# openpsi-project/ReaLHF

Measured on AMD Instinct MI355X. Metric: PPO samples/sec (whole node), 4xLLaMA-7B actor/critic/ref/RM, higher is better.
Workload: dtype bf16; 1 GPU; model=4xllama-7b, global_batch=16, seq_len=640, prompt_len=128, gen_len=512, parallelism=dp1, ppo_n_minibatches=4

## Files before the change

### realhf_amd/ops/csrc/elementwise.hip

```cpp
#include "common.h"

template <typename T, bool CONJ>
__global__ void rope_kernel(
    const T* __restrict__ x, T* __restrict__ out,
    const float* __restrict__ cosb, const float* __restrict__ sinb,
    const long* __restrict__ pos, int total, int nh, int hd) {
  int hd2 = hd / 2;
  long n_quads = (long)total * nh * (hd2 / 4);
  for (long i = (long)blockIdx.x * blockDim.x + threadIdx.x; i < n_quads;
       i += (long)gridDim.x * blockDim.x) {
    int q = i % (hd2 / 4);
    long th = i / (hd2 / 4);
    int h = th % nh;
    long t = th / nh;
    int d0 = q * 4;
    const T* base = x + (t * nh + h) * (long)hd;
    T* obase = out + (t * nh + h) * (long)hd;
    long p = pos[t];
    float4v c = *(const float4v*)(cosb + p * hd2 + d0);
    float4v s = *(const float4v*)(sinb + p * hd2 + d0);
    short4v x1 = *(const short4v*)((const short*)base + d0);
    short4v x2 = *(const short4v*)((const short*)base + hd2 + d0);
    short o1[4], o2[4];
    #pragma unroll
// ... 51 lines not shown
                                  long tokens, int I) {
  long n = tokens * (I / 8);
  for (long i = (long)blockIdx.x * blockDim.x + threadIdx.x; i < n;
       i += (long)gridDim.x * blockDim.x) {
    long t = i / (I / 8);
    int d0 = (int)(i % (I / 8)) * 8;
    const T* g = gu + t * (2L * I) + d0;
    const T* u = g + I;
    short8 gv = *(const short8*)g;
    short8 uv = *(const short8*)u;
    short o[8];
    #pragma unroll
    for (int j = 0; j < 8; j++) {
      float gf = to_f32<T>(((const T*)&gv)[j]);
      float uf = to_f32<T>(((const T*)&uv)[j]);
      float s = gf / (1.f + __expf(-glu_sig_arg<GELU>(gf)));
      ((T*)o)[j] = from_f32<T>(s * uf);
    }
    *(short8*)(out + t * (long)I + d0) = *(short8*)o;
  }
}

template <typename T, bool GELU = false>
__global__ void swiglu_slab_kernel(const float* __restrict__ parts, int nks,
                                   T* __restrict__ out, long tokens, int I) {
  const long sstride = tokens * (2L * I);
  long n = tokens * (I / 8);
  for (long i = (long)blockIdx.x * blockDim.x + threadIdx.x; i < n;
       i += (long)gridDim.x * blockDim.x) {
    long t = i / (I / 8);
    int d0 = (int)(i % (I / 8)) * 8;
    const float* g = parts + t * (2L * I) + d0;
    const float* u = g + I;
    float gf[8], uf[8];
    #pragma unroll
    for (int j = 0; j < 8; j += 4) {
      *(float4v*)(gf + j) = *(const float4v*)(g + j);
      *(float4v*)(uf + j) = *(const float4v*)(u + j);
    }
    for (int s = 1; s < nks; s++) {
      #pragma unroll
      for (int j = 0; j < 8; j += 4) {
        float4v pg = *(const float4v*)(g + (long)s * sstride + j);
        float4v pu = *(const float4v*)(u + (long)s * sstride + j);
        #pragma unroll
        for (int q = 0; q < 4; q++) { gf[j + q] += pg[q]; uf[j + q] += pu[q]; }
      }
    }
    short o[8];
    #pragma unroll
    for (int j = 0; j < 8; j++) {
      float sg = gf[j] / (1.f + __expf(-glu_sig_arg<GELU>(gf[j])));
      ((T*)o)[j] = from_f32<T>(sg * uf[j]);
    }
    *(short8*)(out + t * (long)I + d0) = *(short8*)o;
  }
}

template <typename T, bool GELU = false>
__global__ void swiglu_bwd_kernel(const T* __restrict__ dy, const T* __restrict__ gu,
                                  T* __restrict__ dgu, long tokens, int I) {
  long n = tokens * (I / 8);
  for (long i = (long)blockIdx.x * blockDim.x + threadIdx.x; i < n;
       i += (long)gridDim.x * blockDim.x) {
    long t = i / (I / 8);
    int d0 = (int)(i % (I / 8)) * 8;
    const T* g = gu + t * (2L * I) + d0;
    const T* u = g + I;
    short8 gv = *(const short8*)g;
    short8 uv = *(const short8*)u;
    short8 dv = *(const short8*)(dy + t * (long)I + d0);
    short dg[8], du[8];
    #pragma unroll
    for (int j = 0; j < 8; j++) {
      float gf = to_f32<T>(((const T*)&gv)[j]);
      float uf = to_f32<T>(((const T*)&uv)[j]);
// ... 166 lines not shown
```

### realhf_amd/ops/csrc/rmsnorm.hip

```cpp
#include "common.h"

template <typename T, bool GEMMA>
DEVINL float norm_weight(T w) {
  if constexpr (GEMMA) return 1.0f + to_f32<T>(w);
  else return to_f32<T>(w);
}

template <typename T, int VEC, bool RESID = false, bool GEMMA = false>
__global__ void rmsnorm_fwd_kernel(
    const T* __restrict__ x, const T* __restrict__ w, T* __restrict__ out,
    float* __restrict__ rstd, int rows, int H, float eps,
    const T* __restrict__ resid = nullptr, T* __restrict__ sum_out = nullptr) {
  __shared__ float red[8];
  for (int row = blockIdx.x; row < rows; row += gridDim.x) {
    const T* xr = x + (long)row * H;
    T* yr = out + (long)row * H;
    float ss = 0.f;
    for (int i = threadIdx.x * VEC; i < H; i += blockDim.x * VEC) {
      T v[VEC];
      *(float4v*)v = *(const float4v*)(xr + i);
      if constexpr (RESID) {
        T r[VEC];
        *(float4v*)r = *(const float4v*)(resid + (long)row * H + i);
        #pragma unroll
        for (int j = 0; j < VEC; j++)
          v[j] = from_f32<T>(to_f32<T>(v[j]) + to_f32<T>(r[j]));
        *(float4v*)(sum_out + (long)row * H + i) = *(float4v*)v;
      }
      #pragma unroll
      for (int j = 0; j < VEC; j++) { float f = to_f32<T>(v[j]); ss += f * f; }
    }
    ss = wave_sum(ss);
    int wid = threadIdx.x / WAVE;
    int nw = blockDim.x / WAVE;
    if ((threadIdx.x & (WAVE - 1)) == 0) red[wid] = ss;
    __syncthreads();
    if (threadIdx.x < 8) {
      float v2 = (threadIdx.x < nw) ? red[threadIdx.x] : 0.f;
      for (int off = 4; off > 0; off >>= 1) v2 += __shfl_down(v2, off, 64);
      if (threadIdx.x == 0) red[0] = v2;
    }
    __syncthreads();
    float rs = rsqrtf(red[0] / H + eps);
    if (threadIdx.x == 0 && rstd) rstd[row] = rs;
    const T* src2 = RESID ? (sum_out + (long)row * H) : xr;
    for (int i = threadIdx.x * VEC; i < H; i += blockDim.x * VEC) {
      T v[VEC], wv[VEC], o[VEC];
      *(float4v*)v = *(const float4v*)(src2 + i);
      *(float4v*)wv = *(const float4v*)(w + i);
      #pragma unroll
      for (int j = 0; j < VEC; j++)
        o[j] = from_f32<T>(to_f32<T>(v[j]) * rs * norm_weight<T, GEMMA>(wv[j]));
      *(float4v*)(yr + i) = *(float4v*)o;
    }
    __syncthreads();
  }
}

template <typename T, int VEC, bool GEMMA = false>
__global__ void add_rmsnorm_slab_kernel(
    const float* __restrict__ parts, int nks, const T* __restrict__ resid,
    const T* __restrict__ w, T* __restrict__ out, T* __restrict__ sum_out,
    int rows, int H, float eps) {
  __shared__ float red[8];
  const long sstride = (long)rows * H;
  for (int row = blockIdx.x; row < rows; row += gridDim.x) {
// ... 4 lines not shown
      const float* pr = parts + (long)row * H + i;
      #pragma unroll
      for (int j = 0; j < VEC; j += 4)
        *(float4v*)(f + j) = *(const float4v*)(pr + j);
      for (int s = 1; s < nks; s++) {
        #pragma unroll
        for (int j = 0; j < VEC; j += 4) {
          float4v p = *(const float4v*)(pr + (long)s * sstride + j);
          #pragma unroll
          for (int q = 0; q < 4; q++) f[j + q] += p[q];
        }
      }
      T r[VEC], v[VEC];
      *(float4v*)r = *(const float4v*)(resid + (long)row * H + i);
      #pragma unroll
      for (int j = 0; j < VEC; j++) {
        float fv = f[j] + to_f32<T>(r[j]);
        v[j] = from_f32<T>(fv);
        float fq = to_f32<T>(v[j]);
        ss += fq * fq;
      }
      *(float4v*)(sum_out + (long)row * H + i) = *(float4v*)v;
    }
    ss = wave_sum(ss);
    int wid = threadIdx.x / WAVE;
    int nw = blockDim.x / WAVE;
    if ((threadIdx.x & (WAVE - 1)) == 0) red[wid] = ss;
    __syncthreads();
    if (threadIdx.x < 8) {
      float v2 = (threadIdx.x < nw) ? red[threadIdx.x] : 0.f;
      for (int off = 4; off > 0; off >>= 1) v2 += __shfl_down(v2, off, 64);
      if (threadIdx.x == 0) red[0] = v2;
    }
    __syncthreads();
    float rs = rsqrtf(red[0] / H + eps);
    const T* src2 = sum_out + (long)row * H;
    for (int i = threadIdx.x * VEC; i < H; i += blockDim.x * VEC) {
      T v[VEC], wv[VEC], o[VEC];
      *(float4v*)v = *(const float4v*)(src2 + i);
      *(float4v*)wv = *(const float4v*)(w + i);
      #pragma unroll
      for (int j = 0; j < VEC; j++)
        o[j] = from_f32<T>(to_f32<T>(v[j]) * rs * norm_weight<T, GEMMA>(wv[j]));
      *(float4v*)(yr + i) = *(float4v*)o;
    }
    __syncthreads();
  }
}

#define RMS_MAX_COLS 64
#define RMS_THREADS 256

template <typename T, int VEC, bool GEMMA = false>
__global__ void __launch_bounds__(GEMMA ? RMS_THREADS : 1024) rmsnorm_bwd_kernel(
    const T* __restrict__ dy, const T* __restrict__ x, const T* __restrict__ w,
    const float* __restrict__ rstd, T* __restrict__ dx,
    float* __restrict__ dw, int rows, int H) {
  __shared__ float red[8];
  float dwacc[RMS_MAX_COLS];
  #pragma unroll
  for (int j = 0; j < RMS_MAX_COLS; j++) dwacc[j] = 0.f;
  for (int row = blockIdx.x; row < rows; row += gridDim.x) {
    const T* dyr = dy + (long)row * H;
    const T* xr = x + (long)row * H;
    T* dxr = dx + (long)row * H;
    float rs = rstd[row];
    float dot = 0.f;
    for (int i = threadIdx.x * VEC; i < H; i += blockDim.x * VEC) {
      T a[VEC], b[VEC], c[VEC];
      *(float4v*)a = *(const float4v*)(dyr + i);
      *(float4v*)b = *(const float4v*)(w + i);
      *(float4v*)c = *(const float4v*)(xr + i);
      #pragma unroll
      for (int j = 0; j < VEC; j++)
        dot += to_f32<T>(a[j]) * norm_weight<T, GEMMA>(b[j]) * to_f32<T>(c[j]);
    }
    dot = wave_sum(dot);
    int wid = threadIdx.x / WAVE, nw = blockDim.x / WAVE;
    if ((threadIdx.x & (WAVE - 1)) == 0) red[wid] = dot;
    __syncthreads();
    if (threadIdx.x < 8) {
      float v2 = (threadIdx.x < nw) ? red[threadIdx.x] : 0.f;
      for (int off = 4; off > 0; off >>= 1) v2 += __shfl_down(v2, off, 64);
      if (threadIdx.x == 0) red[0] = v2;
    }
    __syncthreads();
    float k = red[0] * rs * rs * rs / H;
    if constexpr (GEMMA) {
      #pragma unroll
      for (int c = 0; c < RMS_MAX_COLS / VEC; c++) {
        int i = (c * RMS_THREADS + (int)threadIdx.x) * VEC;
        if (i >= H) continue;
        T a[VEC], b[VEC], cx[VEC], o[VEC];
        *(float4v*)a = *(const float4v*)(dyr + i);
        *(float4v*)b = *(const float4v*)(w + i);
        *(float4v*)cx = *(const float4v*)(xr + i);
        #pragma unroll
        for (int j = 0; j < VEC; j++) {
          float g = to_f32<T>(a[j]);
          float xv = to_f32<T>(cx[j]);
          o[j] = from_f32<T>(rs * norm_weight<T, true>(b[j]) * g - k * xv);
          dwacc[c * VEC + j] += g * xv * rs;
        }
        *(float4v*)(dxr + i) = *(float4v*)o;
      }
    } else {
      int slot = 0;
      for (int i = threadIdx.x * VEC; i < H; i += blockDim.x * VEC, slot += VEC) {
        T a[VEC], b[VEC], c[VEC], o[VEC];
        *(float4v*)a = *(const float4v*)(dyr + i);
// ... 21 lines not shown
      for (int j = 0; j < VEC; j++) dwrow[i + j] = dwacc[c * VEC + j];
    }
  } else {
    int slot = 0;
    for (int i = threadIdx.x * VEC; i < H; i += blockDim.x * VEC, slot += VEC) {
      #pragma unroll
      for (int j = 0; j < VEC; j++)
        if (slot + j < RMS_MAX_COLS) dwrow[i + j] = dwacc[slot + j];
    }
  }
}

template <bool GEMMA>
static std::vector<torch::Tensor> rmsnorm_fwd_impl(torch::Tensor x, torch::Tensor w,
                                                   double eps) {
  TORCH_CHECK(x.is_cuda() && x.is_contiguous());
  int H = x.size(-1);
  long rows = x.numel() / H;
  auto out = torch::empty_like(x);
  auto rstd = torch::empty({rows}, x.options().dtype(torch::kFloat));
  int vec = 16 / x.element_size();
  TORCH_CHECK(H % vec == 0, "hidden dim must be divisible by ", vec);
  int grid = (int)std::min<long>(rows, 2048);
  DISPATCH_BF16_FP16_FP32(x.scalar_type(), "rmsnorm_fwd", [&] {
    if (x.element_size() == 2) {
      hipLaunchKernelGGL((rmsnorm_fwd_kernel<scalar_t, 8, false, GEMMA>), dim3(grid), dim3(256), 0,
        cur_stream(), (const scalar_t*)x.data_ptr(), (const scalar_t*)w.data_ptr(),
        (scalar_t*)out.data_ptr(), rstd.data_ptr<float>(), (int)rows, H, (float)eps);
    } else {
      hipLaunchKernelGGL((rmsnorm_fwd_kernel<scalar_t, 4, false, GEMMA>), dim3(grid), dim3(256), 0,
        cur_stream(), (const scalar_t*)x.data_ptr(), (const scalar_t*)w.data_ptr(),
        (scalar_t*)out.data_ptr(), rstd.data_ptr<float>(), (int)rows, H, (float)eps);
    }
  });
  CHECK_CUDA_OK();
  return {out, rstd};
}

template <bool GEMMA>
static std::vector<torch::Tensor> add_rmsnorm_fwd_impl(torch::Tensor x,
                                                       torch::Tensor resid,
                                                       torch::Tensor w, double eps) {
  TORCH_CHECK(x.is_cuda() && x.is_contiguous() && resid.is_contiguous());
  int H = x.size(-1);
  long rows = resid.numel() / H;
  TORCH_CHECK(H % 8 == 0);
  auto out = torch::empty_like(resid);
  auto sum_out = torch::empty_like(resid);
  int grid = (int)std::min<long>(rows, 2048);
  if (x.dim() == 3 && x.scalar_type() == torch::kFloat) {
    TORCH_CHECK(resid.scalar_type() == torch::kBFloat16);
    TORCH_CHECK(x.size(1) * x.size(2) == rows * H);
    hipLaunchKernelGGL((add_rmsnorm_slab_kernel<bf16, 8, GEMMA>), dim3(grid),
      dim3(256), 0, cur_stream(), x.data_ptr<float>(), (int)x.size(0),
      (const bf16*)resid.data_ptr(), (const bf16*)w.data_ptr(),
      (bf16*)out.data_ptr(), (bf16*)sum_out.data_ptr(), (int)rows, H,
      (float)eps);
    CHECK_CUDA_OK();
    return {out, sum_out};
  }
  TORCH_CHECK(x.element_size() == 2);
  DISPATCH_BF16_FP16_FP32(x.scalar_type(), "add_rmsnorm", [&] {
    if constexpr (sizeof(scalar_t) == 2) {
      hipLaunchKernelGGL((rmsnorm_fwd_kernel<scalar_t, 8, true, GEMMA>), dim3(grid),
        dim3(256), 0, cur_stream(), (const scalar_t*)x.data_ptr(),
        (const scalar_t*)w.data_ptr(), (scalar_t*)out.data_ptr(),
        nullptr, (int)rows, H, (float)eps,
        (const scalar_t*)resid.data_ptr(), (scalar_t*)sum_out.data_ptr());
    }
  });
  CHECK_CUDA_OK();
  return {out, sum_out};
}

template <bool GEMMA>
static std::vector<torch::Tensor> rmsnorm_bwd_impl(torch::Tensor dy, torch::Tensor x,
                                                   torch::Tensor w,
                                                   torch::Tensor rstd) {
  int H = x.size(-1);
  TORCH_CHECK(H <= 256 * RMS_MAX_COLS, "rmsnorm_bwd supports hidden <= 16384");
  long rows = x.numel() / H;
  auto dx = torch::empty_like(x);
  int grid = (int)std::min<long>(rows, 512);
  auto dw32 = torch::zeros({grid, H}, x.options().dtype(torch::kFloat));
  DISPATCH_BF16_FP16_FP32(x.scalar_type(), "rmsnorm_bwd", [&] {
    if (x.element_size() == 2) {
      hipLaunchKernelGGL((rmsnorm_bwd_kernel<scalar_t, 8, GEMMA>), dim3(grid), dim3(RMS_THREADS), 0,
        cur_stream(), (const scalar_t*)dy.data_ptr(), (const scalar_t*)x.data_ptr(),
        (const scalar_t*)w.data_ptr(), rstd.data_ptr<float>(),
        (scalar_t*)dx.data_ptr(), dw32.data_ptr<float>(), (int)rows, H);
    } else {
// ... 34 lines not shown
```

### realhf_amd/ops/csrc/rope_decode.hip

```cpp
#include "common.h"
#include "fp8_e4m3.h"

template <bool SLAB, int FP8_HD = 0>
__global__ void rope_qkv_decode_kernel(
    const void* __restrict__ qkv_in,
    const bf16* __restrict__ bias,
    bf16* __restrict__ q_out,
    void* __restrict__ kcache,
    void* __restrict__ vcache,
    float* __restrict__ kscale,
    float* __restrict__ vscale,
    const int* __restrict__ cache_seqlens,
    const float* __restrict__ cosb, const float* __restrict__ sinb,
    int bs, int nq, int nkv, int hd, long maxlen, long qkv_stride,
    bool apply_rope, int nks) {
  const int nh = nq + 2 * nkv;
  const int hd2 = hd / 2;
  const long nwork = (long)bs * nh * (hd2 / 4);
  for (long i = (long)blockIdx.x * blockDim.x + threadIdx.x; i < nwork;
       i += (long)gridDim.x * blockDim.x) {
    const int quad = i % (hd2 / 4);
    const int h = (i / (hd2 / 4)) % nh;
    const int b = i / ((long)nh * (hd2 / 4));
    const int d0 = quad * 4;
    const int pos = max(cache_seqlens[b] - 1, 0);

    float4v f1, f2;
    if constexpr (SLAB) {
      const float* src =
          (const float*)qkv_in + (long)b * qkv_stride + (long)h * hd;
      const long sstride = (long)bs * qkv_stride;
      f1 = *(const float4v*)(src + d0);
      f2 = *(const float4v*)(src + hd2 + d0);
      for (int s = 1; s < nks; s++) {
        float4v p1 = *(const float4v*)(src + (long)s * sstride + d0);
        float4v p2 = *(const float4v*)(src + (long)s * sstride + hd2 + d0);
        #pragma unroll
        for (int j = 0; j < 4; j++) { f1[j] += p1[j]; f2[j] += p2[j]; }
      }
    } else {
      const bf16* src =
          (const bf16*)qkv_in + (long)b * qkv_stride + (long)h * hd;
      short4v x1 = *(const short4v*)((const short*)src + d0);
      short4v x2 = *(const short4v*)((const short*)src + hd2 + d0);
      #pragma unroll
      for (int j = 0; j < 4; j++) {
        f1[j] = __bfloat162float(((const bf16*)&x1)[j]);
        f2[j] = __bfloat162float(((const bf16*)&x2)[j]);
      }
    }
    if (bias) {
      short4v b1 = *(const short4v*)((const short*)bias + (long)h * hd + d0);
      short4v b2 = *(const short4v*)((const short*)bias + (long)h * hd + hd2 + d0);
      #pragma unroll
      for (int j = 0; j < 4; j++) {
        f1[j] += __bfloat162float(((const bf16*)&b1)[j]);
        f2[j] += __bfloat162float(((const bf16*)&b2)[j]);
      }
    }
    bf16* dst;
    bool rope = apply_rope;
    if (h < nq) {
      dst = q_out + ((long)b * nq + h) * hd;
    } else if (h < nq + nkv) {
      dst = (bf16*)kcache + (((long)b * maxlen + pos) * nkv + (h - nq)) * hd;
    } else {
      dst = (bf16*)vcache +
            (((long)b * maxlen + pos) * nkv + (h - nq - nkv)) * hd;
      rope = false;
    }
    short o1[4], o2[4];
    if (rope) {
      float4v c = *(const float4v*)(cosb + (long)pos * hd2 + d0);
      float4v s = *(const float4v*)(sinb + (long)pos * hd2 + d0);
      #pragma unroll
      for (int j = 0; j < 4; j++) {
        ((bf16*)o1)[j] = __float2bfloat16(f1[j] * c[j] - f2[j] * s[j]);
        ((bf16*)o2)[j] = __float2bfloat16(f2[j] * c[j] + f1[j] * s[j]);
      }
    } else {
      #pragma unroll
      for (int j = 0; j < 4; j++) {
        ((bf16*)o1)[j] = __float2bfloat16(f1[j]);
        ((bf16*)o2)[j] = __float2bfloat16(f2[j]);
      }
    }
    if constexpr (FP8_HD != 0) {
      if (h >= nq) {
        float amax = 0.f;
        #pragma unroll
        for (int j = 0; j < 4; j++)
          amax = fmaxf(amax, fmaxf(fabsf(bf2f(o1[j])), fabsf(bf2f(o2[j]))));
        amax = group_max<FP8_HD / 8>(amax);
        const float sc = e4m3_row_scale(amax);
        const bool is_k = h < nq + nkv;
        const int kvh = is_k ? h - nq : h - nq - nkv;
        unsigned char* cdst =
// ... 111 lines not shown
```

### realhf_amd/ops/csrc/skinny_gemm.hip

```cpp
#include "mfma.h"

#define SG_TN 64

template <int NT>
DEVINL void sg_stage_x(__bf16* x_s, const bf16* __restrict__ x, int M, int K,
                       int k_lo, int k_hi, int kslice) {
  const int kn = k_hi - k_lo;
  for (int idx = threadIdx.x * 8; idx < 16 * kslice; idx += NT * 8) {
    int m = idx / kslice;
    int kk = idx % kslice;
    bf16x8 v = {};
    if (kk < kn && m < M)
      v = *(const bf16x8*)(x + (long)m * K + k_lo + kk);
    *(bf16x8*)(&x_s[(long)m * kslice + kk]) = v;
  }
}

DEVINL void sg_reduce_store(const float* __restrict__ parts, long slab,
                            int nks, long off, const bf16* __restrict__ resid,
                            bf16* __restrict__ out) {
  f32x4 v = *(const f32x4*)(parts + off);
  for (int s = 1; s < nks; s++) {
    f32x4 p = *(const f32x4*)(parts + (long)s * slab + off);
    #pragma unroll
    for (int j = 0; j < 4; j++) v[j] += p[j];
  }
  short o[4];
  if (resid) {
    short4v rv = *(const short4v*)((const short*)resid + off);
    #pragma unroll
    for (int j = 0; j < 4; j++)
      o[j] = f2bf(v[j] + __bfloat162float(((const bf16*)&rv)[j]));
  } else {
    #pragma unroll
    for (int j = 0; j < 4; j++) o[j] = f2bf(v[j]);
  }
  *(short4v*)((short*)out + off) = *(short4v*)o;
}

template <int NB, int WVS = 4>
__global__ __launch_bounds__(64 * WVS, 4) void skinny_gemm_kernel(
    const bf16* __restrict__ x, const bf16* __restrict__ w,
    float* __restrict__ out32, int M, int N, int K, int kslice) {
  const int ntile = blockIdx.x;
  const int ks = blockIdx.y;
  const int k_lo = ks * kslice;
  const int k_hi = min(K, k_lo + kslice);
  const auto [lane, wv, i16, g] = mfma_lane();
  const int n0 = ntile * (WVS * 16) + wv * 16;

  extern __shared__ __bf16 x_s[];
  sg_stage_x<64 * WVS>(x_s, x, M, K, k_lo, k_hi, kslice);
  __syncthreads();

  f32x4 acc[4] = {};
  const bf16* wrow = w + (long)(n0 + i16) * K;
  int kk = k_lo;
  for (; kk + NB * 32 <= k_hi; kk += NB * 32) {
    bf16x8 b[NB], a[NB];
    #pragma unroll
    for (int t = 0; t < NB; t++)
      b[t] = *(const bf16x8*)(wrow + kk + t * 32 + g * 8);
    const long xb = (long)i16 * kslice + (kk - k_lo) + g * 8;
    #pragma unroll
    for (int t = 0; t < NB; t++)
      a[t] = *(const bf16x8*)(&x_s[xb + t * 32]);
    #pragma unroll
    for (int t = 0; t < NB; t++)
      acc[t & 3] = mfma16(a[t], b[t], acc[t & 3]);
  }
  for (; kk + 32 <= k_hi; kk += 32) {
    bf16x8 a0 = *(const bf16x8*)(&x_s[(long)i16 * kslice + (kk - k_lo) + g * 8]);
    bf16x8 b0 = *(const bf16x8*)(wrow + kk + g * 8);
    acc[0] = mfma16(a0, b0, acc[0]);
  }
  #pragma unroll
  for (int r = 0; r < 4; r++) {
    int m = g * 4 + r;
    float vsum = acc[0][r] + acc[1][r] + acc[2][r] + acc[3][r];
    if (m < M)
      out32[((long)ks * M + m) * N + n0 + i16] = vsum;
  }
}

static int sg_depth() {
  static int d = [] {
    const char* e = getenv("REALHF_AMD_SKINNY_DEPTH");
    return (e && e[0] == '8') ? 8 : 4;
  }();
  return d;
}

static int sg_tn32_maxn() {
  static int v = [] {
    const char* e = getenv("REALHF_AMD_SG_TN32_MAXN");
    return e ? atoi(e) : 0;
  }();
  return v;
// ... 179 lines not shown
                           torch::Tensor out32_ws, torch::Tensor sem,
                           long splitk, c10::optional<torch::Tensor> residual) {
  const SgShape s = sg_shape(x, w, out32_ws, splitk);
  TORCH_CHECK(sem.scalar_type() == torch::kInt32 && sem.numel() >= s.N / SG_TN,
              "semaphore buffer too small (must be zero-initialized once)");
  auto out = torch::empty({s.M, (long)s.N}, x.options());
  const bf16* rptr = sg_resid_ptr(residual, (long)s.M * s.N);
  dim3 grid((s.N / SG_TN) * s.nks);
  hipLaunchKernelGGL(skinny_gemm2_kernel, grid, dim3(256), s.lds, cur_stream(),
    (const bf16*)x.data_ptr(), (const bf16*)w.data_ptr(),
    out32_ws.data_ptr<float>(), sem.data_ptr<int>(), rptr,
    (bf16*)out.data_ptr(), s.M, s.N, s.K, s.kslice, s.nks);
  CHECK_CUDA_OK();
  return out;
}

torch::Tensor skinny_gemm(torch::Tensor x, torch::Tensor w,
                          torch::Tensor out32_ws, long splitk,
                          c10::optional<torch::Tensor> residual) {
  const SgShape s = sg_shape(x, w, out32_ws, splitk);
  return sg_combine(sg_partials(x, w, out32_ws, s), x, s, residual);
}

typedef __attribute__((ext_vector_type(4))) int int4v;
typedef __attribute__((ext_vector_type(2))) float float2v;

DEVINL unsigned sg_bf16_pair(float lo, float hi) {
  return (__builtin_bit_cast(unsigned, lo) >> 16) |
         (__builtin_bit_cast(unsigned, hi) & 0xffff0000u);
}

DEVINL bf16x8 sg_e4m3x8_to_bf16(int lo, int hi) {
  const float2v p0 = __builtin_amdgcn_cvt_pk_f32_fp8(lo, false);
  const float2v p1 = __builtin_amdgcn_cvt_pk_f32_fp8(lo, true);
  const float2v p2 = __builtin_amdgcn_cvt_pk_f32_fp8(hi, false);
  const float2v p3 = __builtin_amdgcn_cvt_pk_f32_fp8(hi, true);
  int4v u;
  u[0] = (int)sg_bf16_pair(p0[0], p0[1]);
  u[1] = (int)sg_bf16_pair(p1[0], p1[1]);
  u[2] = (int)sg_bf16_pair(p2[0], p2[1]);
  u[3] = (int)sg_bf16_pair(p3[0], p3[1]);
  return __builtin_bit_cast(bf16x8, u);
}

template <int NB>
__global__ __launch_bounds__(256, 4) void skinny_gemm_fp8_kernel(
    const bf16* __restrict__ x, const unsigned char* __restrict__ q,
    const float* __restrict__ scale, float* __restrict__ out32, int M, int N,
    int K, int kslice) {
  const int ntile = blockIdx.x;
  const int ks = blockIdx.y;
  const int k_lo = ks * kslice;
  const int k_hi = min(K, k_lo + kslice);
  const auto [lane, wv, i16, g] = mfma_lane();
  const int n0 = ntile * SG_TN + wv * 16;

  extern __shared__ __bf16 x_s[];
  sg_stage_x<256>(x_s, x, M, K, k_lo, k_hi, kslice);
  __syncthreads();

  f32x4 acc[4] = {};
  const unsigned char* qrow = q + (long)(n0 + i16) * K + g * 16;
  const int xo = i16 * kslice + g * 16 - k_lo;
  int kk = k_lo;
  for (; kk + NB * 64 <= k_hi; kk += NB * 64) {
    int4v b[NB];
    #pragma unroll
    for (int t = 0; t < NB; t++)
      b[t] = *(const int4v*)(qrow + kk + t * 64);
    bf16x8 a[2 * NB];
    #pragma unroll
    for (int t = 0; t < NB; t++) {
      a[2 * t] = *(const bf16x8*)(&x_s[xo + kk + t * 64]);
      a[2 * t + 1] = *(const bf16x8*)(&x_s[xo + kk + t * 64 + 8]);
    }
    #pragma unroll
    for (int t = 0; t < NB; t++) {
      acc[(2 * t) & 3] = mfma16(a[2 * t], sg_e4m3x8_to_bf16(b[t][0], b[t][1]),
                                acc[(2 * t) & 3]);
      acc[(2 * t + 1) & 3] = mfma16(a[2 * t + 1],
                                    sg_e4m3x8_to_bf16(b[t][2], b[t][3]),
                                    acc[(2 * t + 1) & 3]);
    }
  }
  for (; kk + 64 <= k_hi; kk += 64) {
    const int4v b0 = *(const int4v*)(qrow + kk);
    const bf16x8 a0 = *(const bf16x8*)(&x_s[xo + kk]);
    const bf16x8 a1 = *(const bf16x8*)(&x_s[xo + kk + 8]);
    acc[0] = mfma16(a0, sg_e4m3x8_to_bf16(b0[0], b0[1]), acc[0]);
    acc[1] = mfma16(a1, sg_e4m3x8_to_bf16(b0[2], b0[3]), acc[1]);
  }
  const float sc = scale[n0 + i16];
  #pragma unroll
  for (int r = 0; r < 4; r++) {
    int m = g * 4 + r;
    float vsum = acc[0][r] + acc[1][r] + acc[2][r] + acc[3][r];
    if (m < M)
      out32[((long)ks * M + m) * N + n0 + i16] = vsum * sc;
  }
}

static SgShape sg_shape_fp8(const torch::Tensor& x, const torch::Tensor& q,
                            const torch::Tensor& scale,
                            const torch::Tensor& out32_ws, long splitk) {
  TORCH_CHECK(q.is_cuda() && q.dim() == 2 && q.element_size() == 1 &&
              q.is_contiguous() && (uintptr_t)q.data_ptr() % 16 == 0,
              "q must be contiguous, 16-byte aligned [N, K] e4m3 bytes");
  TORCH_CHECK(x.dim() == 2 && x.size(1) == q.size(1), "x / q K mismatch");
  TORCH_CHECK(q.size(1) % 64 == 0, "fp8 skinny GEMM needs K % 64 == 0");
  TORCH_CHECK(scale.is_cuda() && scale.scalar_type() == torch::kFloat32 &&
              scale.is_contiguous() && scale.numel() == q.size(0),
              "scale must be contiguous fp32 [N]");
  TORCH_CHECK(out32_ws.is_cuda() && out32_ws.scalar_type() == torch::kFloat32);
  return sg_shape(x, q, out32_ws, splitk);
}
// ... 31 lines not shown
```

Before: 3.660 samples/s.

## Batch split-K slab loads, add single-pass row RMSNorm, double-buffer skinny GEMM weights

Adds a shared slab_sum helper that issues several split-K partial loads before accumulating, replacing serial per-slab loops in the SwiGLU, RoPE decode, GEMM reduce and RMSNorm paths. Adds a one-block-per-row RMSNorm kernel that keeps the row in registers for small decode batches (rows ≤ 16), which avoids re-reading it from memory. Restructures the bf16 and fp8 skinny GEMM main loops to double-buffer weight loads and overlap the x staging with the first weight fetch. These target memory latency in decode-time kernels, at the cost of higher register pressure and more template code.

```diff
diff --git a/realhf_amd/ops/csrc/elementwise.hip b/realhf_amd/ops/csrc/elementwise.hip
--- a/realhf_amd/ops/csrc/elementwise.hip
+++ b/realhf_amd/ops/csrc/elementwise.hip
@@ -1,4 +1,5 @@
 #include "common.h"
+#include "slab_sum.h"
 
 template <typename T, bool CONJ>
 __global__ void rope_kernel(
@@ -97,8 +98,9 @@
 }
 
 template <typename T, bool GELU = false>
-__global__ void swiglu_slab_kernel(const float* __restrict__ parts, int nks,
-                                   T* __restrict__ out, long tokens, int I) {
+__global__ __launch_bounds__(256) void swiglu_slab_kernel(
+    const float* __restrict__ parts, int nks, T* __restrict__ out, long tokens,
+    int I) {
   const long sstride = tokens * (2L * I);
   long n = tokens * (I / 8);
   for (long i = (long)blockIdx.x * blockDim.x + threadIdx.x; i < n;
@@ -107,26 +109,15 @@
     int d0 = (int)(i % (I / 8)) * 8;
     const float* g = parts + t * (2L * I) + d0;
     const float* u = g + I;
-    float gf[8], uf[8];
-    #pragma unroll
-    for (int j = 0; j < 8; j += 4) {
-      *(float4v*)(gf + j) = *(const float4v*)(g + j);
-      *(float4v*)(uf + j) = *(const float4v*)(u + j);
-    }
-    for (int s = 1; s < nks; s++) {
-      #pragma unroll
-      for (int j = 0; j < 8; j += 4) {
-        float4v pg = *(const float4v*)(g + (long)s * sstride + j);
-        float4v pu = *(const float4v*)(u + (long)s * sstride + j);
-        #pragma unroll
-        for (int q = 0; q < 4; q++) { gf[j + q] += pg[q]; uf[j + q] += pu[q]; }
-      }
-    }
+    const float* const p[4] = {g, g + 4, u, u + 4};
+    float4v acc[4];
+    slab_sum<4>(acc, p, sstride, nks);
     short o[8];
     #pragma unroll
     for (int j = 0; j < 8; j++) {
-      float sg = gf[j] / (1.f + __expf(-glu_sig_arg<GELU>(gf[j])));
-      ((T*)o)[j] = from_f32<T>(sg * uf[j]);
+      const float gf = acc[j / 4][j % 4], uf = acc[2 + j / 4][j % 4];
+      float sg = gf / (1.f + __expf(-glu_sig_arg<GELU>(gf)));
+      ((T*)o)[j] = from_f32<T>(sg * uf);
     }
     *(short8*)(out + t * (long)I + d0) = *(short8*)o;
   }
diff --git a/realhf_amd/ops/csrc/rmsnorm.hip b/realhf_amd/ops/csrc/rmsnorm.hip
--- a/realhf_amd/ops/csrc/rmsnorm.hip
+++ b/realhf_amd/ops/csrc/rmsnorm.hip
@@ -1,9 +1,25 @@
 #include "common.h"
+#include "slab_sum.h"
 
 template <typename T, bool GEMMA>
 DEVINL float norm_weight(T w) {
   if constexpr (GEMMA) return 1.0f + to_f32<T>(w);
   else return to_f32<T>(w);
+}
+
+DEVINL float rms_block_sum(float v, float* red) {
+  v = wave_sum(v);
+  int wid = threadIdx.x / WAVE;
+  int nw = blockDim.x / WAVE;
+  if ((threadIdx.x & (WAVE - 1)) == 0) red[wid] = v;
+  __syncthreads();
+  if (threadIdx.x < 8) {
+    float v2 = (threadIdx.x < nw) ? red[threadIdx.x] : 0.f;
+    for (int off = 4; off > 0; off >>= 1) v2 += __shfl_down(v2, off, 64);
+    if (threadIdx.x == 0) red[0] = v2;
+  }
+  __syncthreads();
+  return red[0];
 }
 
 template <typename T, int VEC, bool RESID = false, bool GEMMA = false>
@@ -30,18 +46,7 @@
       #pragma unroll
       for (int j = 0; j < VEC; j++) { float f = to_f32<T>(v[j]); ss += f * f; }
     }
-    ss = wave_sum(ss);
-    int wid = threadIdx.x / WAVE;
-    int nw = blockDim.x / WAVE;
-    if ((threadIdx.x & (WAVE - 1)) == 0) red[wid] = ss;
-    __syncthreads();
-    if (threadIdx.x < 8) {
-      float v2 = (threadIdx.x < nw) ? red[threadIdx.x] : 0.f;
-      for (int off = 4; off > 0; off >>= 1) v2 += __shfl_down(v2, off, 64);
-      if (threadIdx.x == 0) red[0] = v2;
-    }
-    __syncthreads();
-    float rs = rsqrtf(red[0] / H + eps);
+    float rs = rsqrtf(rms_block_sum(ss, red) / H + eps);
     if (threadIdx.x == 0 && rstd) rstd[row] = rs;
     const T* src2 = RESID ? (sum_out + (long)row * H) : xr;
     for (int i = threadIdx.x * VEC; i < H; i += blockDim.x * VEC) {
@@ -92,18 +97,7 @@
       }
       *(float4v*)(sum_out + (long)row * H + i) = *(float4v*)v;
     }
-    ss = wave_sum(ss);
-    int wid = threadIdx.x / WAVE;
-    int nw = blockDim.x / WAVE;
-    if ((threadIdx.x & (WAVE - 1)) == 0) red[wid] = ss;
-    __syncthreads();
-    if (threadIdx.x < 8) {
-      float v2 = (threadIdx.x < nw) ? red[threadIdx.x] : 0.f;
-      for (int off = 4; off > 0; off >>= 1) v2 += __shfl_down(v2, off, 64);
-      if (threadIdx.x == 0) red[0] = v2;
-    }
-    __syncthreads();
-    float rs = rsqrtf(red[0] / H + eps);
+    float rs = rsqrtf(rms_block_sum(ss, red) / H + eps);
     const T* src2 = sum_out + (long)row * H;
     for (int i = threadIdx.x * VEC; i < H; i += blockDim.x * VEC) {
       T v[VEC], wv[VEC], o[VEC];
@@ -118,8 +112,108 @@
   }
 }
 
+#define RMS_THREADS 256
+#define RMS_ROW_MAX_ROWS 16
+#define RMS_ROW_MAX_NP 4
+enum { RMS_SRC_PLAIN, RMS_SRC_RESID, RMS_SRC_SLAB };
+
+template <typename T, int VEC, int NP, int SRC, bool GEMMA>
+__global__ __launch_bounds__(RMS_THREADS) void rmsnorm_row_kernel(
+    const void* __restrict__ xin,
+    int nks, const T* __restrict__ resid, const T* __restrict__ w,
+    T* __restrict__ out, T* __restrict__ sum_out, float* __restrict__ rstd,
+    int rows, int H, float eps) {
+  __shared__ float red[8];
+  const long ro = (long)blockIdx.x * H;
+  bool on[NP];
+  int col[NP];
+  #pragma unroll
+  for (int c = 0; c < NP; c++) {
+    const int i = (c * RMS_THREADS + (int)threadIdx.x) * VEC;
+    on[c] = i < H;
+    col[c] = on[c] ? i : 0;
+  }
+  T wv[NP][VEC], r[NP][VEC], v[NP][VEC];
+  #pragma unroll
+  for (int c = 0; c < NP; c++)
+    *(float4v*)wv[c] = *(const float4v*)(w + col[c]);
+  if constexpr (SRC != RMS_SRC_PLAIN) {
+    #pragma unroll
+    for (int c = 0; c < NP; c++)
+      *(float4v*)r[c] = *(const float4v*)(resid + ro + col[c]);
+  }
+  if constexpr (SRC == RMS_SRC_SLAB) {
+    static_assert(VEC == 8, "two float4 per thread and pass");
+    const float* p[2 * NP];
+    #pragma unroll
+    for (int c = 0; c < NP; c++) {
+      p[2 * c] = (const float*)xin + ro + col[c];
+      p[2 * c + 1] = p[2 * c] + 4;
+    }
+    float4v acc[2 * NP];
+    slab_sum<2 * NP, (NP > 2 ? 4 : SLAB_BATCH)>(
+        acc, (const float* const (&)[2 * NP])p, (long)rows * H, nks);
+    #pragma unroll
+    for (int c = 0; c < NP; c++) {
+      #pragma unroll
+      for (int j = 0; j < VEC; j++)
+        v[c][j] = from_f32<T>(acc[2 * c + j / 4][j % 4] + to_f32<T>(r[c][j]));
+    }
+  } else {
+    #pragma unroll
+    for (int c = 0; c < NP; c++)
+      *(float4v*)v[c] = *(const float4v*)((const T*)xin + ro + col[c]);
+    if constexpr (SRC == RMS_SRC_RESID) {
+      #pragma unroll
+      for (int c = 0; c < NP; c++) {
+        #pragma unroll
+        for (int j = 0; j < VEC; j++)
+          v[c][j] = from_f32<T>(to_f32<T>(v[c][j]) + to_f32<T>(r[c][j]));
+      }
+    }
+  }
+  float ss = 0.f;
+  #pragma unroll
+  for (int c = 0; c < NP; c++) {
+    if (!on[c]) continue;
+    if constexpr (SRC != RMS_SRC_PLAIN)
+      *(float4v*)(sum_out + ro + col[c]) = *(float4v*)v[c];
+    #pragma unroll
+    for (int j = 0; j < VEC; j++) { float f = to_f32<T>(v[c][j]); ss += f * f; }
+  }
+  float rs = rsqrtf(rms_block_sum(ss, red) / H + eps);
+  if (threadIdx.x == 0 && rstd) rstd[blockIdx.x] = rs;
+  #pragma unroll
+  for (int c = 0; c < NP; c++) {
+    if (!on[c]) continue;
+    T o[VEC];
+    #pragma unroll
+    for (int j = 0; j < VEC; j++)
+      o[j] = from_f32<T>(to_f32<T>(v[c][j]) * rs * norm_weight<T, GEMMA>(wv[c][j]));
+    *(float4v*)(out + ro + col[c]) = *(float4v*)o;
+  }
+}
+
+static bool rms_row_gate(long rows, int H, int vec) {
+  return rows <= RMS_ROW_MAX_ROWS && H <= RMS_THREADS * vec * RMS_ROW_MAX_NP;
+}
+
+template <typename T, int VEC, int SRC, bool GEMMA>
+static void rms_row_launch(const void* xin, int nks, const T* resid, const T* w,
+                           T* out, T* sum_out, float* rstd, int rows, int H,
+                           float eps) {
+  auto go = [&](auto np) {
+    hipLaunchKernelGGL((rmsnorm_row_kernel<T, VEC, np.value, SRC, GEMMA>),
+      dim3(rows), dim3(RMS_THREADS), 0, cur_stream(), xin, nks, resid, w, out,
+      sum_out, rstd, rows, H, eps);
+  };
+  const int per = RMS_THREADS * VEC;
+  if (H <= per) go(std::integral_constant<int, 1>{});
+  else if (H <= 2 * per) go(std::integral_constant<int, 2>{});
+  else go(std::integral_constant<int, 4>{});
+}
+
 #define RMS_MAX_COLS 64
-#define RMS_THREADS 256
 
 template <typename T, int VEC, bool GEMMA = false>
 __global__ void __launch_bounds__(GEMMA ? RMS_THREADS : 1024) rmsnorm_bwd_kernel(
@@ -145,17 +239,7 @@
       for (int j = 0; j < VEC; j++)
         dot += to_f32<T>(a[j]) * norm_weight<T, GEMMA>(b[j]) * to_f32<T>(c[j]);
     }
-    dot = wave_sum(dot);
-    int wid = threadIdx.x / WAVE, nw = blockDim.x / WAVE;
-    if ((threadIdx.x & (WAVE - 1)) == 0) red[wid] = dot;
-    __syncthreads();
-    if (threadIdx.x < 8) {
-      float v2 = (threadIdx.x < nw) ? red[threadIdx.x] : 0.f;
-      for (int off = 4; off > 0; off >>= 1) v2 += __shfl_down(v2, off, 64);
-      if (threadIdx.x == 0) red[0] = v2;
-    }
-    __syncthreads();
-    float k = red[0] * rs * rs * rs / H;
+    float k = rms_block_sum(dot, red) * rs * rs * rs / H;
     if constexpr (GEMMA) {
       #pragma unroll
       for (int c = 0; c < RMS_MAX_COLS / VEC; c++) {
@@ -223,8 +307,15 @@
   int vec = 16 / x.element_size();
   TORCH_CHECK(H % vec == 0, "hidden dim must be divisible by ", vec);
   int grid = (int)std::min<long>(rows, 2048);
+  const bool few = x.element_size() == 2 && rms_row_gate(rows, H, vec);
   DISPATCH_BF16_FP16_FP32(x.scalar_type(), "rmsnorm_fwd", [&] {
-    if (x.element_size() == 2) {
+    if (few) {
+      if constexpr (sizeof(scalar_t) == 2)
+        rms_row_launch<scalar_t, 8, RMS_SRC_PLAIN, GEMMA>(
+          x.data_ptr(), 1, nullptr, (const scalar_t*)w.data_ptr(),
+          (scalar_t*)out.data_ptr(), nullptr, rstd.data_ptr<float>(),
+          (int)rows, H, (float)eps);
+    } else if (x.element_size() == 2) {
       hipLaunchKernelGGL((rmsnorm_fwd_kernel<scalar_t, 8, false, GEMMA>), dim3(grid), dim3(256), 0,
         cur_stream(), (const scalar_t*)x.data_ptr(), (const scalar_t*)w.data_ptr(),
         (scalar_t*)out.data_ptr(), rstd.data_ptr<float>(), (int)rows, H, (float)eps);
@@ -252,22 +343,34 @@
   if (x.dim() == 3 && x.scalar_type() == torch::kFloat) {
     TORCH_CHECK(resid.scalar_type() == torch::kBFloat16);
     TORCH_CHECK(x.size(1) * x.size(2) == rows * H);
-    hipLaunchKernelGGL((add_rmsnorm_slab_kernel<bf16, 8, GEMMA>), dim3(grid),
-      dim3(256), 0, cur_stream(), x.data_ptr<float>(), (int)x.size(0),
-      (const bf16*)resid.data_ptr(), (const bf16*)w.data_ptr(),
-      (bf16*)out.data_ptr(), (bf16*)sum_out.data_ptr(), (int)rows, H,
-      (float)eps);
+    if (rms_row_gate(rows, H, 8))
+      rms_row_launch<bf16, 8, RMS_SRC_SLAB, GEMMA>(
+        x.data_ptr(), (int)x.size(0), (const bf16*)resid.data_ptr(),
+        (const bf16*)w.data_ptr(), (bf16*)out.data_ptr(),
+        (bf16*)sum_out.data_ptr(), nullptr, (int)rows, H, (float)eps);
+    else
+      hipLaunchKernelGGL((add_rmsnorm_slab_kernel<bf16, 8, GEMMA>), dim3(grid),
+        dim3(256), 0, cur_stream(), x.data_ptr<float>(), (int)x.size(0),
+        (const bf16*)resid.data_ptr(), (const bf16*)w.data_ptr(),
+        (bf16*)out.data_ptr(), (bf16*)sum_out.data_ptr(), (int)rows, H,
+        (float)eps);
     CHECK_CUDA_OK();
     return {out, sum_out};
   }
   TORCH_CHECK(x.element_size() == 2);
   DISPATCH_BF16_FP16_FP32(x.scalar_type(), "add_rmsnorm", [&] {
     if constexpr (sizeof(scalar_t) == 2) {
-      hipLaunchKernelGGL((rmsnorm_fwd_kernel<scalar_t, 8, true, GEMMA>), dim3(grid),
-        dim3(256), 0, cur_stream(), (const scalar_t*)x.data_ptr(),
-        (const scalar_t*)w.data_ptr(), (scalar_t*)out.data_ptr(),
-        nullptr, (int)rows, H, (float)eps,
-        (const scalar_t*)resid.data_ptr(), (scalar_t*)sum_out.data_ptr());
+      if (rms_row_gate(rows, H, 8))
+        rms_row_launch<scalar_t, 8, RMS_SRC_RESID, GEMMA>(
+          x.data_ptr(), 1, (const scalar_t*)resid.data_ptr(),
+          (const scalar_t*)w.data_ptr(), (scalar_t*)out.data_ptr(),
+          (scalar_t*)sum_out.data_ptr(), nullptr, (int)rows, H, (float)eps);
+      else
+        hipLaunchKernelGGL((rmsnorm_fwd_kernel<scalar_t, 8, true, GEMMA>), dim3(grid),
+          dim3(256), 0, cur_stream(), (const scalar_t*)x.data_ptr(),
+          (const scalar_t*)w.data_ptr(), (scalar_t*)out.data_ptr(),
+          nullptr, (int)rows, H, (float)eps,
+          (const scalar_t*)resid.data_ptr(), (scalar_t*)sum_out.data_ptr());
     }
   });
   CHECK_CUDA_OK();
diff --git a/realhf_amd/ops/csrc/rope_decode.hip b/realhf_amd/ops/csrc/rope_decode.hip
--- a/realhf_amd/ops/csrc/rope_decode.hip
+++ b/realhf_amd/ops/csrc/rope_decode.hip
@@ -1,8 +1,9 @@
 #include "common.h"
 #include "fp8_e4m3.h"
+#include "slab_sum.h"
 
 template <bool SLAB, int FP8_HD = 0>
-__global__ void rope_qkv_decode_kernel(
+__global__ __launch_bounds__(256) void rope_qkv_decode_kernel(
     const void* __restrict__ qkv_in,
     const bf16* __restrict__ bias,
     bf16* __restrict__ q_out,
@@ -25,19 +26,25 @@
     const int d0 = quad * 4;
     const int pos = max(cache_seqlens[b] - 1, 0);
 
+    short4v b1 = {}, b2 = {};
+    float4v c = {}, s = {};
+    if (bias) {
+      b1 = *(const short4v*)((const short*)bias + (long)h * hd + d0);
+      b2 = *(const short4v*)((const short*)bias + (long)h * hd + hd2 + d0);
+    }
+    if (apply_rope) {
+      c = *(const float4v*)(cosb + (long)pos * hd2 + d0);
+      s = *(const float4v*)(sinb + (long)pos * hd2 + d0);
+    }
     float4v f1, f2;
     if constexpr (SLAB) {
       const float* src =
           (const float*)qkv_in + (long)b * qkv_stride + (long)h * hd;
-      const long sstride = (long)bs * qkv_stride;
-      f1 = *(const float4v*)(src + d0);
-      f2 = *(const float4v*)(src + hd2 + d0);
-      for (int s = 1; s < nks; s++) {
-        float4v p1 = *(const float4v*)(src + (long)s * sstride + d0);
-        float4v p2 = *(const float4v*)(src + (long)s * sstride + hd2 + d0);
-        #pragma unroll
-        for (int j = 0; j < 4; j++) { f1[j] += p1[j]; f2[j] += p2[j]; }
-      }
+      const float* const p[2] = {src + d0, src + hd2 + d0};
+      float4v acc[2];
+      slab_sum<2>(acc, p, (long)bs * qkv_stride, nks);
+      f1 = acc[0];
+      f2 = acc[1];
     } else {
       const bf16* src =
           (const bf16*)qkv_in + (long)b * qkv_stride + (long)h * hd;
@@ -50,8 +57,6 @@
       }
     }
     if (bias) {
-      short4v b1 = *(const short4v*)((const short*)bias + (long)h * hd + d0);
-      short4v b2 = *(const short4v*)((const short*)bias + (long)h * hd + hd2 + d0);
       #pragma unroll
       for (int j = 0; j < 4; j++) {
         f1[j] += __bfloat162float(((const bf16*)&b1)[j]);
@@ -71,8 +76,6 @@
     }
     short o1[4], o2[4];
     if (rope) {
-      float4v c = *(const float4v*)(cosb + (long)pos * hd2 + d0);
-      float4v s = *(const float4v*)(sinb + (long)pos * hd2 + d0);
       #pragma unroll
       for (int j = 0; j < 4; j++) {
         ((bf16*)o1)[j] = __float2bfloat16(f1[j] * c[j] - f2[j] * s[j]);
diff --git a/realhf_amd/ops/csrc/skinny_gemm.hip b/realhf_amd/ops/csrc/skinny_gemm.hip
--- a/realhf_amd/ops/csrc/skinny_gemm.hip
+++ b/realhf_amd/ops/csrc/skinny_gemm.hip
@@ -1,4 +1,5 @@
 #include "mfma.h"
+#include "slab_sum.h"
 
 #define SG_TN 64
 
@@ -19,15 +20,14 @@
 DEVINL void sg_reduce_store(const float* __restrict__ parts, long slab,
                             int nks, long off, const bf16* __restrict__ resid,
                             bf16* __restrict__ out) {
-  f32x4 v = *(const f32x4*)(parts + off);
-  for (int s = 1; s < nks; s++) {
-    f32x4 p = *(const f32x4*)(parts + (long)s * slab + off);
-    #pragma unroll
-    for (int j = 0; j < 4; j++) v[j] += p[j];
-  }
+  short4v rv = {};
+  if (resid) rv = *(const short4v*)((const short*)resid + off);
+  const float* const p[1] = {parts + off};
+  f32x4 acc[1];
+  slab_sum<1>(acc, p, slab, nks);
+  const f32x4 v = acc[0];
   short o[4];
   if (resid) {
-    short4v rv = *(const short4v*)((const short*)resid + off);
     #pragma unroll
     for (int j = 0; j < 4; j++)
       o[j] = f2bf(v[j] + __bfloat162float(((const bf16*)&rv)[j]));
@@ -36,6 +36,157 @@
     for (int j = 0; j < 4; j++) o[j] = f2bf(v[j]);
   }
   *(short4v*)((short*)out + off) = *(short4v*)o;
+}
+
+typedef __attribute__((ext_vector_type(4))) int int4v;
+typedef __attribute__((ext_vector_type(2))) float float2v;
+
+DEVINL bf16x8 sg_e4m3x8_to_bf16(int lo, int hi);
+
+#define SG_XV 8
+
+template <int NT>
+DEVINL void sg_x_load(bf16x8 (&v)[SG_XV], const bf16* __restrict__ x, int M,
+                      int K, int k_lo, int k_hi, int kslice) {
+  const int kn = k_hi - k_lo;
+  const int dm = (NT * 8) / kslice, dk = (NT * 8) % kslice;
+  int m = (threadIdx.x * 8) / kslice;
+  int kk = (threadIdx.x * 8) % kslice;
+  #pragma unroll
+  for (int t = 0; t < SG_XV; t++) {
+    const bool ok = kk < kn && m < M;
+    const bf16* p = ok ? x + (long)m * K + k_lo + kk : x;
+    const bf16x8 r = *(const bf16x8*)p;
+    v[t] = ok ? r : bf16x8{};
+    m += dm;
+    kk += dk;
+    if (kk >= kslice) { kk -= kslice; m++; }
+  }
+}
+
+template <int NT>
+DEVINL void sg_x_store(__bf16* x_s, const bf16x8 (&v)[SG_XV],
+                       const bf16* __restrict__ x, int M, int K, int k_lo,
+                       int k_hi, int kslice) {
+  #pragma unroll
+  for (int t = 0; t < SG_XV; t++) {
+    const int idx = (threadIdx.x + t * NT) * 8;
+    if (idx < 16 * kslice) *(bf16x8*)(&x_s[idx]) = v[t];
+  }
+  const int kn = k_hi - k_lo;
+  for (int idx = (threadIdx.x + SG_XV * NT) * 8; idx < 16 * kslice;
+       idx += NT * 8) {
+    int m = idx / kslice;
+    int kk = idx % kslice;
+    bf16x8 r = {};
+    if (kk < kn && m < M)
+      r = *(const bf16x8*)(x + (long)m * K + k_lo + kk);
+    *(bf16x8*)(&x_s[idx]) = r;
+  }
+}
+
+template <bool FP8>
+struct SgLane {
+  static constexpr int KB = FP8 ? 64 : 32;
+  const char* wl;
+  const __bf16* x_s;
+  int xo;
+
+  DEVINL int4v ldw(int k) const {
+    return *(const int4v*)(wl + (long)k * (FP8 ? 1 : 2));
+  }
+  DEVINL void mma(f32x4 (&acc)[4], const int4v& b, int k, int j) const {
+    if constexpr (FP8) {
+      const bf16x8 a0 = *(const bf16x8*)(&x_s[xo + k]);
+      const bf16x8 a1 = *(const bf16x8*)(&x_s[xo + k + 8]);
+      acc[(2 * j) & 3] = mfma16(a0, sg_e4m3x8_to_bf16(b[0], b[1]),
+                                acc[(2 * j) & 3]);
+      acc[(2 * j + 1) & 3] = mfma16(a1, sg_e4m3x8_to_bf16(b[2], b[3]),
+                                    acc[(2 * j + 1) & 3]);
+    } else {
+      const bf16x8 a0 = *(const bf16x8*)(&x_s[xo + k]);
+      acc[j & 3] = mfma16(a0, __builtin_bit_cast(bf16x8, b), acc[j & 3]);
+    }
+  }
+  template <int NB>
+  DEVINL void ldw_batch(int4v (&b)[NB], int k) const {
+    #pragma unroll
+    for (int t = 0; t < NB; t++) b[t] = ldw(k + t * KB);
+    __builtin_amdgcn_sched_barrier(0);
+  }
+  template <int NB>
+  DEVINL void mma_batch(f32x4 (&acc)[4], const int4v (&b)[NB], int k) const {
+    #pragma unroll
+    for (int t = 0; t < NB; t++) mma(acc, b[t], k + t * KB, t);
+  }
+};
+
+template <bool FP8, int NB, int NTL>
+DEVINL void sg_finish(const SgLane<FP8>& ln, f32x4 (&acc)[4],
+                      const int4v (&last)[NB], bool has_last, int k) {
+  constexpr int KB = SgLane<FP8>::KB;
+  const int kt = has_last ? k + NB * KB : k;
+  int4v tb[NTL > 0 ? NTL : 1];
+  #pragma unroll
+  for (int t = 0; t < NTL; t++) tb[t] = ln.ldw(kt + t * KB);
+  __builtin_amdgcn_sched_barrier(0);
+  if (has_last) ln.template mma_batch<NB>(acc, last, k);
+  #pragma unroll
+  for (int t = 0; t < NTL; t++) ln.mma(acc, tb[t], kt + t * KB, 0);
+}
+
+template <bool FP8, int NB, int NTL = 0>
+DEVINL void sg_finish_n(const SgLane<FP8>& ln, f32x4 (&acc)[4],
+                        const int4v (&last)[NB], bool has_last, int k,
+                        int ntail) {
+  if (ntail == NTL) sg_finish<FP8, NB, NTL>(ln, acc, last, has_last, k);
+  else if constexpr (NTL + 2 < NB)
+    sg_finish_n<FP8, NB, NTL + 1>(ln, acc, last, has_last, k, ntail);
+  else sg_finish<FP8, NB, NB - 1>(ln, acc, last, has_last, k);
+}
+
+template <bool FP8, int NB, int NT>
+DEVINL void sg_slice(f32x4 (&acc)[4], __bf16* x_s, const bf16* __restrict__ x,
+                     const void* __restrict__ wrow, int g, int i16, int M,
+                     int K, int k_lo, int k_hi, int kslice) {
+  constexpr int KB = SgLane<FP8>::KB;
+  constexpr int S = NB * KB;
+  SgLane<FP8> ln;
+  ln.wl = (const char*)wrow + g * 16;
+  ln.x_s = x_s;
+  ln.xo = i16 * kslice + g * (KB / 4) - k_lo;
+  int nb = (k_hi - k_lo) / S;
+  const int ntail = ((k_hi - k_lo) - nb * S) / KB;
+
+  bf16x8 xv[SG_XV];
+  sg_x_load<NT>(xv, x, M, K, k_lo, k_hi, kslice);
+  int4v b0[NB], b1[NB];
+  int kk = k_lo;
+  #pragma unroll
+  for (int t = 0; t < NB; t++) b0[t] = ln.ldw(nb > 0 ? kk + t * KB : kk);
+  __builtin_amdgcn_sched_barrier(0);
+  sg_x_store<NT>(x_s, xv, x, M, K, k_lo, k_hi, kslice);
+  __syncthreads();
+
+  if (nb == 0) {
+    sg_finish_n<FP8, NB>(ln, acc, b0, false, kk, ntail);
+    return;
+  }
+  while (nb > 2) {
+    ln.template ldw_batch<NB>(b1, kk + S);
+    ln.template mma_batch<NB>(acc, b0, kk);
+    ln.template ldw_batch<NB>(b0, kk + 2 * S);
+    ln.template mma_batch<NB>(acc, b1, kk + S);
+    kk += 2 * S;
+    nb -= 2;
+  }
+  if (nb == 2) {
+    ln.template ldw_batch<NB>(b1, kk + S);
+    ln.template mma_batch<NB>(acc, b0, kk);
+    sg_finish_n<FP8, NB>(ln, acc, b1, true, kk + S, ntail);
+  } else {
+    sg_finish_n<FP8, NB>(ln, acc, b0, true, kk, ntail);
+  }
 }
 
 template <int NB, int WVS = 4>
@@ -50,30 +201,9 @@
   const int n0 = ntile * (WVS * 16) + wv * 16;
 
   extern __shared__ __bf16 x_s[];
-  sg_stage_x<64 * WVS>(x_s, x, M, K, k_lo, k_hi, kslice);
-  __syncthreads();
-
   f32x4 acc[4] = {};
-  const bf16* wrow = w + (long)(n0 + i16) * K;
-  int kk = k_lo;
-  for (; kk + NB * 32 <= k_hi; kk += NB * 32) {
-    bf16x8 b[NB], a[NB];
-    #pragma unroll
-    for (int t = 0; t < NB; t++)
-      b[t] = *(const bf16x8*)(wrow + kk + t * 32 + g * 8);
-    const long xb = (long)i16 * kslice + (kk - k_lo) + g * 8;
-    #pragma unroll
-    for (int t = 0; t < NB; t++)
-      a[t] = *(const bf16x8*)(&x_s[xb + t * 32]);
-    #pragma unroll
-    for (int t = 0; t < NB; t++)
-      acc[t & 3] = mfma16(a[t], b[t], acc[t & 3]);
-  }
-  for (; kk + 32 <= k_hi; kk += 32) {
-    bf16x8 a0 = *(const bf16x8*)(&x_s[(long)i16 * kslice + (kk - k_lo) + g * 8]);
-    bf16x8 b0 = *(const bf16x8*)(wrow + kk + g * 8);
-    acc[0] = mfma16(a0, b0, acc[0]);
-  }
+  sg_slice<false, NB, 64 * WVS>(acc, x_s, x, w + (long)(n0 + i16) * K, g, i16,
+                                M, K, k_lo, k_hi, kslice);
   #pragma unroll
   for (int r = 0; r < 4; r++) {
     int m = g * 4 + r;
@@ -299,9 +429,6 @@
   return sg_combine(sg_partials(x, w, out32_ws, s), x, s, residual);
 }
 
-typedef __attribute__((ext_vector_type(4))) int int4v;
-typedef __attribute__((ext_vector_type(2))) float float2v;
-
 DEVINL unsigned sg_bf16_pair(float lo, float hi) {
   return (__builtin_bit_cast(unsigned, lo) >> 16) |
          (__builtin_bit_cast(unsigned, hi) & 0xffff0000u);
@@ -333,41 +460,10 @@
   const int n0 = ntile * SG_TN + wv * 16;
 
   extern __shared__ __bf16 x_s[];
-  sg_stage_x<256>(x_s, x, M, K, k_lo, k_hi, kslice);
-  __syncthreads();
-
+  const float sc = scale[n0 + i16];
   f32x4 acc[4] = {};
-  const unsigned char* qrow = q + (long)(n0 + i16) * K + g * 16;
-  const int xo = i16 * kslice + g * 16 - k_lo;
-  int kk = k_lo;
-  for (; kk + NB * 64 <= k_hi; kk += NB * 64) {
-    int4v b[NB];
-    #pragma unroll
-    for (int t = 0; t < NB; t++)
-      b[t] = *(const int4v*)(qrow + kk + t * 64);
-    bf16x8 a[2 * NB];
-    #pragma unroll
-    for (int t = 0; t < NB; t++) {
-      a[2 * t] = *(const bf16x8*)(&x_s[xo + kk + t * 64]);
-      a[2 * t + 1] = *(const bf16x8*)(&x_s[xo + kk + t * 64 + 8]);
-    }
-    #pragma unroll
-    for (int t = 0; t < NB; t++) {
-      acc[(2 * t) & 3] = mfma16(a[2 * t], sg_e4m3x8_to_bf16(b[t][0], b[t][1]),
-                                acc[(2 * t) & 3]);
-      acc[(2 * t + 1) & 3] = mfma16(a[2 * t + 1],
-                                    sg_e4m3x8_to_bf16(b[t][2], b[t][3]),
-                                    acc[(2 * t + 1) & 3]);
-    }
-  }
-  for (; kk + 64 <= k_hi; kk += 64) {
-    const int4v b0 = *(const int4v*)(qrow + kk);
-    const bf16x8 a0 = *(const bf16x8*)(&x_s[xo + kk]);
-    const bf16x8 a1 = *(const bf16x8*)(&x_s[xo + kk + 8]);
-    acc[0] = mfma16(a0, sg_e4m3x8_to_bf16(b0[0], b0[1]), acc[0]);
-    acc[1] = mfma16(a1, sg_e4m3x8_to_bf16(b0[2], b0[3]), acc[1]);
-  }
-  const float sc = scale[n0 + i16];
+  sg_slice<true, NB, 256>(acc, x_s, x, q + (long)(n0 + i16) * K, g, i16, M, K,
+                          k_lo, k_hi, kslice);
   #pragma unroll
   for (int r = 0; r < 4; r++) {
     int m = g * 4 + r;
diff --git a/realhf_amd/ops/csrc/slab_sum.h b/realhf_amd/ops/csrc/slab_sum.h
--- /dev/null
+++ b/realhf_amd/ops/csrc/slab_sum.h
@@ -0,0 +1,54 @@
+#pragma once
+#include "common.h"
+
+#define SLAB_BATCH 8
+
+template <int NB, int NV, bool FIRST>
+DEVINL void slab_batch(float4v (&acc)[NV], const float* const (&p)[NV],
+                       long sstride, int s0) {
+  float4v b[NB][NV];
+  #pragma unroll
+  for (int t = 0; t < NB; t++) {
+    #pragma unroll
+    for (int v = 0; v < NV; v++)
+      b[t][v] = *(const float4v*)(p[v] + (long)(s0 + t) * sstride);
+  }
+  #pragma unroll
+  for (int t = 0; t < NB; t++) {
+    #pragma unroll
+    for (int v = 0; v < NV; v++) {
+      if (FIRST && t == 0) acc[v] = b[0][v];
+      else acc[v] += b[t][v];
+    }
+  }
+}
+
+template <int MAXB, int NV, bool FIRST>
+DEVINL void slab_rem(float4v (&acc)[NV], const float* const (&p)[NV],
+                     long sstride, int s0, int n) {
+  static_assert(MAXB <= 8, "slab_rem lists batches of up to 7");
+  switch (n) {
+    case 1: slab_batch<1, NV, FIRST>(acc, p, sstride, s0); break;
+    case 2: slab_batch<2, NV, FIRST>(acc, p, sstride, s0); break;
+    case 3: slab_batch<3, NV, FIRST>(acc, p, sstride, s0); break;
+    case 4: if constexpr (MAXB > 4) slab_batch<4, NV, FIRST>(acc, p, sstride, s0); break;
+    case 5: if constexpr (MAXB > 4) slab_batch<5, NV, FIRST>(acc, p, sstride, s0); break;
+    case 6: if constexpr (MAXB > 4) slab_batch<6, NV, FIRST>(acc, p, sstride, s0); break;
+    case 7: if constexpr (MAXB > 4) slab_batch<7, NV, FIRST>(acc, p, sstride, s0); break;
+  }
+}
+
+template <int NV, int MAXB = SLAB_BATCH>
+DEVINL void slab_sum(float4v (&acc)[NV], const float* const (&p)[NV],
+                     long sstride, int nks) {
+  static_assert(MAXB == 4 || MAXB == 8, "batch depth 4 or 8");
+  if (nks < MAXB) {
+    slab_rem<MAXB, NV, true>(acc, p, sstride, 0, nks);
+    return;
+  }
+  slab_batch<MAXB, NV, true>(acc, p, sstride, 0);
+  int s = MAXB;
+  for (; s + MAXB <= nks; s += MAXB)
+    slab_batch<MAXB, NV, false>(acc, p, sstride, s);
+  if (s < nks) slab_rem<MAXB, NV, false>(acc, p, sstride, s, nks - s);
+}
```

New measurement: 3.859 samples/s, median of 6. 5.4% higher.
